# CaptainCuong/Efficient-GNN

Measured on NVIDIA B200. Metric: chebyshev_wavelet_nnz_k_f_per_s, higher is better.
Workload: dtype f32

## Files before the change

efficient-gnn_b200/_cabi.py:

```python
from __future__ import annotations

import ctypes as C
import os
import threading

_HERE = os.path.dirname(os.path.abspath(__file__))
LIB_PATH = os.environ.get("EGNN_LIB_PATH") or os.path.join(_HERE, "lib", "libegnn_b200.so")
ABI_VERSION = 8

_P, _I32, _I64, _F32, _SZ = C.c_void_p, C.c_int32, C.c_int64, C.c_float, C.c_size_t
SYMBOLS = {
    "egnn_abi_version": (C.c_int, []),
    "egnn_last_error": (C.c_char_p, []),
    "egnn_device_info": (C.c_int, [_P, _P, _P]),
    "egnn_dense_to_csr_count": (C.c_int, [_P, _I64, _I64, _P, _P, _P]),
    "egnn_dense_to_csr_fill": (C.c_int, [_P, _I64, _I64, _P, _P, _P, _P]),
    "egnn_graph_prep": (C.c_int, [_P, _P, _P, _I64, _P, _P, _P, _P, _P, _P, _P, _P, _P]),
    "egnn_degree_rows": (C.c_int, [_P, _P, _P, _I64, _I64, _I64, _P, _P, _P, _P, _P]),
    "egnn_graph_prep_finish": (C.c_int, [_P, _P, _P, _I64, _P, _P, _P, _P, _P]),
    "egnn_calibration_metrics_ws_bytes": (_SZ, [_I32, _I32]),
    "egnn_calibration_metrics": (C.c_int, [_P, _I32, _P, _P, _I64, _I32, _I32, _P, _P, _SZ, _P]),
    "egnn_temperature_head": (C.c_int, [_P, _P, _P, _P, _P, _P, _P, _P, _I64, _I32, _I32, _I32, _P]),
    "egnn_gcn_propagate": (C.c_int, [_P, _P, _P, _P, _P, _P, _P, _I64, _I32, _P, _P, _P, _I32, _P]),
    "egnn_gcn_target_logits": (C.c_int, [_P, _P, _P, _P, _P, _P, _I32, _I64, _I32, _I32, _P, _P, _P, _P, _P, _I32, _P]),
    "egnn_gcn_structure_grad": (C.c_int, [_P, _P, _P, _P, _P, _P, _P, _P, _P, _P, _I32, _I64, _I32, _I32, _P, _P,
                                          _P, _P, _P, _I32, _P]),
    "egnn_sell_geometry": (C.c_int, [_I64, _I64, _P, _P, _P]),
    "egnn_sell_ws_bytes": (_SZ, [_I64, _I64, _I32, _I32]),
    "egnn_sell_prepare": (C.c_int, [_P, _P, _I64, _I64, _P, _P, _SZ, _P]),
    "egnn_sell_fill": (C.c_int, [_P, _P, _I64, _I64, _P, _P, _SZ, _P]),
    "egnn_patch_degrees": (C.c_int, [_P, _P, _P, _P, _P, _I64, _P, _P, _P, _I32, _P, _P, _P, _I64, _I64, _P]),
# ... 22 lines not shown
                                         _F32, _F32, _I32, _P, _P, _P, _I32, _P, _P, _I32, _P, _P]),
    "egnn_peer_window_bytes": (_SZ, [_I64, _I32, _I32]),
    "egnn_peer_alloc": (C.c_int, [_SZ, _P, _P]),
    "egnn_peer_open": (C.c_int, [_P, _P]),
    "egnn_peer_close": (C.c_int, [_P]),
    "egnn_peer_free": (C.c_int, [_P]),
    "egnn_peer_operand": (_P, [_P, _I32]),
    "egnn_peer_error": (C.c_int, [_P, _P, _P]),
    "egnn_peer_wait_stats": (C.c_int, [_P, _P, _P, _I32, _P]),
    "egnn_peer_prescale_push": (C.c_int, [_P, _P, _I64, _I64, _I32, _P, _P]),
    "egnn_wide_order_sharded": (C.c_int, [_P, _P, _P, _P, _P, _P, _P, _P, _P, _I64, _I64, _I64, _I32, _I32, _I32, _I32,
                                          _P, _F32, _F32, _I32, _P, _P, _P, _I32, _P, _P]),
    "egnn_prescale": (C.c_int, [_P, _P, _P, _I64, _I32, _I64, _P]),
    "egnn_graph_prep_sharded": (C.c_int, [_P, _P, _P, _I64, _I64, _I64, _I32, _P, _P, _P, _P, _P, _P, _P, _P, _P]),
    "egnn_cheb_order_sharded": (C.c_int, [_P, _P, _P, _P, _P, _P, _P, _P, _P, _P, _P, _P,
                                          _I64, _I64, _I64, _I64, _I32, _I32, _I32, _I32, _P, _F32, _F32,
                                          _I32, _I32, _P, _P, _P, _I32, _P]),
}


class SellPlanStruct(C.Structure):
    _fields_ = [("n", C.c_int32), ("n_blocks", C.c_int32), ("col_block", C.c_int32), ("lmax", C.c_int32),
                ("n_cols", C.c_int32), ("row0", C.c_int32), ("n_cta", C.c_int32), ("reserved", C.c_int32),
                ("n_slices", C.c_int64), ("n_vrows", C.c_int64), ("n_entries", C.c_int64), ("n_rowv", C.c_int64),
                ("slice_off", C.c_void_p), ("blk_slice_ptr", C.c_void_p), ("idx", C.c_void_p),
                ("rv_ptr", C.c_void_p), ("vslot", C.c_void_p), ("cta_info", C.c_void_p), ("vpart", C.c_void_p),
                ("sched", C.c_void_p), ("stamps", C.c_void_p)]


MAX_RANKS = 16
IPC_HANDLE_BYTES = 64


class PeerWindowStruct(C.Structure):
    _fields_ = [("rank", C.c_int32), ("world", C.c_int32), ("rows_per", C.c_int64), ("f", C.c_int32),
                ("reserved", C.c_int32), ("base", C.c_void_p * MAX_RANKS)]


class EgnnError(RuntimeError):
    """A non-zero status from libegnn_b200 (message from egnn_last_error)."""


_lock = threading.Lock()
_lib = None


# ... 68 lines not shown
```

efficient-gnn_b200/csrc/egnn_cabi.cu:

```cuda
#include <stdarg.h>
#include <stdlib.h>

#include "adjoint.cuh"
#include "cheb.cuh"
#include "common.cuh"
#include "head.cuh"
#include "metrics.cuh"
#include "peer.cuh"
#include "prep.cuh"
#include "sell.cuh"
#include "sell_step.cuh"
#include "structure_grad.cuh"
#include "surrogate.cuh"
#include "blocked.cuh"
#include "wide.cuh"

namespace egnn {

static thread_local char g_err[512] = {0};
char* last_error_buf() { return g_err; }
void set_error(const char* fmt, ...) {
    va_list ap;
    va_start(ap, fmt);
    vsnprintf(g_err, sizeof(g_err), fmt, ap);
// ... 216 lines not shown
    EGNN_REQUIRE(w->world >= 1 && w->world <= EGNN_MAX_RANKS && w->rank >= 0 && w->rank < w->world, "bad rank/world");
    EGNN_REQUIRE(w->rows_per >= 1 && w->f >= 1, "bad window shape");
    for (int r = 0; r < w->world; ++r) EGNN_REQUIRE(w->base[r] != nullptr, "window of a rank is not mapped");
    return EGNN_OK;
}
static void fill_peer_push(PeerPush& pp, const egnn_peer_window* w, int which, bool has_data, bool wait_first) {
    pp.world = w->world; pp.rank = w->rank; pp.wait_first = wait_first; pp.has_data = has_data;
    char* own = (char*)w->base[w->rank];
    for (int r = 0; r < w->world; ++r) {
        pp.dst[r] = peer_operand(w, r, which);
        pp.flag[r] = (unsigned*)((char*)w->base[r] + kPeerFlagsOff) + w->rank;
    }
    pp.local_flags = (unsigned*)(own + kPeerFlagsOff);
    pp.epoch = (unsigned*)(own + kPeerEpochOff);
    pp.done_ctr = (unsigned*)(own + kPeerDoneOff);
    pp.error = (unsigned*)(own + kPeerErrorOff);
}

static void step_fill_plan(SellStepParams& sp, const egnn_sell_plan* pl) {
    sp.idx = pl->idx; sp.slice_off = pl->slice_off; sp.blk_slice_ptr = pl->blk_slice_ptr; sp.vslot = pl->vslot;
    sp.cta_info = pl->cta_info; sp.rv_ptr = pl->rv_ptr; sp.vpart = pl->vpart; sp.sched = pl->sched;
    sp.stamps = (unsigned long long*)pl->stamps;
    sp.trace = pl->reserved;
    sp.n_cta = pl->n_cta; sp.C = pl->n_blocks; sp.CB = pl->col_block; sp.n_cols = pl->n_cols;
    sp.n_rows = pl->n; sp.row0 = pl->row0;
}

static void step_fill_peer(SellStepParams& sp, const egnn_peer_window* w) {
    sp.world = w->world; sp.rank = w->rank; sp.rows_per = w->rows_per;
    char* own = (char*)w->base[w->rank];
    for (int r = 0; r < w->world; ++r) sp.flag_at[r] = (unsigned*)((char*)w->base[r] + kPeerFlagsOff) + w->rank;
    sp.local_flags = (unsigned*)(own + kPeerFlagsOff);
    sp.epoch = (unsigned*)(own + kPeerEpochOff);
    sp.error = (unsigned*)(own + kPeerErrorOff);
}

static int launch_sell_step(const SellStepParams& sp, bool peer, cudaStream_t st) {
    const size_t smem = sizeof(float) * ((size_t)sp.CB + kSellZeroSlots);
    const bool patch = sp.w_base != nullptr && sp.delta.n > 0;
    const void* fn = peer ? (patch ? (const void*)sell_step_kernel<true, true> : (const void*)sell_step_kernel<true, false>)
                          : (patch ? (const void*)sell_step_kernel<false, true> : (const void*)sell_step_kernel<false, false>);
    int rc = check_cuda(cudaFuncSetAttribute(fn, cudaFuncAttributeMaxDynamicSharedMemorySize, (int)smem),
                        "cudaFuncSetAttribute(sell_step_kernel)");
    if (rc) return rc;
    cudaLaunchConfig_t cfg = {};
    cfg.gridDim = dim3((unsigned)sp.n_cta, 1, 1);
    cfg.blockDim = dim3(kSellThreads, 1, 1);
    cfg.dynamicSmemBytes = smem;
    cfg.stream = st;
    cudaLaunchAttribute attr[1];
    attr[0].id = cudaLaunchAttributeCooperative;
    attr[0].val.cooperative = 1;
    cfg.attrs = attr;
    cfg.numAttrs = 1;
    void* args[1] = {(void*)&sp};
    return check_cuda(cudaLaunchKernelExC(&cfg, fn, args), "sell_step_kernel launch");
}

static int run_sell_step(SellStepParams sp, int k, int n_scales, const float* coeffs_host, bool peer, cudaStream_t st,
                         int order_begin = 1, int order_end = -1) {
    if (order_end < 0) order_end = k;
    const float* held = sp.operand_first;
    for (int ob = order_begin; ob <= order_end; ob += kStepMaxOrders) {
        const int oe = ob + kStepMaxOrders - 1 < order_end ? ob + kStepMaxOrders - 1 : order_end;
        sp.order_begin = ob; sp.order_end = oe; sp.k_max = k; sp.S = n_scales;
        sp.operand_first = ob == order_begin ? held : nullptr;
        for (int s = 0; s < n_scales; ++s)
            for (int j = 0; j <= oe - ob + 1; ++j) sp.coef[s][j] = coeffs_host[s * (k + 1) + ob - 1 + j];
        int rc = launch_sell_step(sp, peer, st);
        if (rc) return rc;
    }
    return EGNN_OK;
}

static int device_sm_count() {
    int dev = 0, sms = kSmCountB200;
    if (cudaGetDevice(&dev) == cudaSuccess) cudaDeviceGetAttribute(&sms, cudaDevAttrMultiProcessorCount, dev);
    return sms;
}

}

using namespace egnn;

extern "C" {

int egnn_abi_version(void) { return 8; }

const char* egnn_last_error(void) { return last_error_buf(); }

int egnn_device_info(int32_t* sm_count, int32_t* cc_major, int32_t* cc_minor) {
    int dev = 0;
    int rc = check_cuda(cudaGetDevice(&dev), "cudaGetDevice");
    if (rc) return rc;
    cudaDeviceProp prop;
    rc = check_cuda(cudaGetDeviceProperties(&prop, dev), "cudaGetDeviceProperties");
    if (rc) return rc;
    if (sm_count) *sm_count = prop.multiProcessorCount;
    if (cc_major) *cc_major = prop.major;
    if (cc_minor) *cc_minor = prop.minor;
    if (prop.major != 10) {
        set_error("libegnn_b200 is built for sm_100a only; device is sm_%d%d", prop.major, prop.minor);
        return EGNN_ERR_UNSUPPORTED_ARCH;
    }
    return EGNN_OK;
}

int egnn_dense_to_csr_count(const float* adj, int64_t n, int64_t ld, int32_t* rowptr,
                            int32_t* nonbinary, egnn_stream_t stream) {
    EGNN_REQUIRE(adj && rowptr && nonbinary, "null pointer");
// ... 844 lines not shown

int egnn_sell_geometry(int64_t n, int64_t nnz, int32_t* n_blocks, int32_t* col_block, int32_t* lmax) {
    EGNN_REQUIRE(n_blocks && col_block && lmax, "null pointer");
    EGNN_REQUIRE(n >= 1, "bad shape");
    int nb = 1, cb = 32;
    narrow_geometry(n, &nb, &cb);
    *n_blocks = nb;
    *col_block = cb;
    *lmax = 256;
    (void)nnz;
    return EGNN_OK;
}

size_t egnn_sell_ws_bytes(int64_t n, int64_t nnz, int32_t n_blocks, int32_t lmax) {
    if (n < 1 || n_blocks < 1 || lmax < 8) return 0;
    return sell_ws_layout(nullptr, n, nnz, n_blocks, lmax).total_bytes;
}

int egnn_sell_prepare(const int32_t* rowptr, const int32_t* colidx, int64_t n, int64_t nnz,
                      egnn_sell_plan* plan, void* workspace, size_t workspace_bytes, egnn_stream_t stream) {
    int rc = sell_check_geometry(n, nnz, plan);
    if (rc) return rc;
    EGNN_REQUIRE(rowptr && (colidx || nnz == 0), "null pointer");
    const int C = plan->n_blocks, CB = plan->col_block, lmax = plan->lmax;
    SellWs w = sell_ws_layout(workspace, n, nnz, C, lmax);
    if (!workspace || workspace_bytes < w.total_bytes) {
        set_error("sell workspace too small: need %zu bytes, got %zu", w.total_bytes, workspace_bytes);
        return EGNN_ERR_WORKSPACE;
    }
    cudaStream_t st = (cudaStream_t)stream;
    const int64_t cn = (int64_t)C * n;
    rc = check_cuda(cudaMemsetAsync(w.nv + cn, 0, 4, st), "memset"); if (rc) return rc;
    rc = check_cuda(cudaMemsetAsync(w.nvrow + n, 0, 4, st), "memset"); if (rc) return rc;
    rc = check_cuda(cudaMemsetAsync(w.key, 0xff, 4 * w.umax, st), "memset"); if (rc) return rc;
    rc = check_cuda(cudaMemsetAsync(w.slice_sz, 0, 4 * (w.smax + 1), st), "memset"); if (rc) return rc;
    rc = check_cuda(cudaMemsetAsync(w.totals, 0, 64, st), "memset"); if (rc) return rc;
    sell_count_kernel<<<(unsigned)ceil_div64(n, 256), 256, 0, st>>>(rowptr, colidx, (int)n, C, CB, lmax, w.seg_start,
                                                                   w.seg_cnt, w.nv, w.nvrow);
    EGNN_LAUNCH_CHECK("sell_count_kernel launch");
    size_t tb = w.cub_bytes;
    rc = check_cuda(cub::DeviceScan::ExclusiveSum(w.cub_temp, tb, w.nv, w.u_off, (int)(cn + 1), st), "scan nv"); if (rc) return rc;
    tb = w.cub_bytes;
    rc = check_cuda(cub::DeviceScan::ExclusiveSum(w.cub_temp, tb, w.nvrow, w.rv_ptr, (int)(n + 1), st), "scan nvrow"); if (rc) return rc;
    sell_emit_kernel<<<(unsigned)ceil_div64(cn, 256), 256, 0, st>>>((int)n, C, lmax, w.seg_start, w.seg_cnt, w.nv, w.u_off,
                                                                   w.rv_ptr, w.key, w.uval, w.vsrc, w.vslot, w.vrow);
    EGNN_LAUNCH_CHECK("sell_emit_kernel launch");
    tb = w.cub_bytes;
    rc = check_cuda(cub::DeviceRadixSort::SortPairs(w.cub_temp, tb, w.key, w.key_sorted, w.uval, w.perm, (int)w.umax, 0, 32, st), "sort vrows");
    if (rc) return rc;
    sell_blocks_kernel<<<1, 32, 0, st>>>((int)n, C, w.u_off, w.q_ptr, w.vp_ptr, w.bsp, w.bstride, w.totals);
    EGNN_LAUNCH_CHECK("sell_blocks_kernel launch");
    sell_slice_kernel<<<(unsigned)ceil_div64(w.smax, 256), 256, 0, st>>>(C, lmax, w.key_sorted, w.q_ptr, w.bsp, w.bstride, w.totals, w.slice_sz);
    EGNN_LAUNCH_CHECK("sell_slice_kernel launch");
    tb = w.cub_bytes;
    rc = check_cuda(cub::DeviceScan::ExclusiveSum(w.cub_temp, tb, w.slice_sz, w.slice_off, (int)(w.smax + 1), st), "scan slices"); if (rc) return rc;
    sell_totals_kernel<<<1, 32, 0, st>>>(w.slice_off, w.rv_ptr, (int)n, w.totals);
    EGNN_LAUNCH_CHECK("sell_totals_kernel launch");
    int64_t tot[8];
    rc = check_cuda(cudaMemcpyAsync(tot, w.totals, 64, cudaMemcpyDeviceToHost, st), "copy totals"); if (rc) return rc;
    rc = check_cuda(cudaStreamSynchronize(st), "sync"); if (rc) return rc;
    plan->n = (int32_t)n;
    plan->n_cta = device_sm_count();
    plan->n_vrows = tot[kTotV];
    plan->n_slices = tot[kTotSlices];
    plan->n_entries = tot[kTotEntries];
    plan->n_rowv = tot[kTotRowV];
    return EGNN_OK;
}

int egnn_sell_fill(const int32_t* rowptr, const int32_t* colidx, int64_t n, int64_t nnz,
                   const egnn_sell_plan* plan, void* workspace, size_t workspace_bytes, egnn_stream_t stream) {
    int rc = sell_check_geometry(n, nnz, plan);
    if (rc) return rc;
    (void)rowptr;
    EGNN_REQUIRE(plan->slice_off && plan->blk_slice_ptr && plan->rv_ptr && plan->cta_info && plan->sched, "plan buffers not allocated");
    EGNN_REQUIRE(plan->n_cta >= 1 && plan->n_cta <= 4096, "n_cta out of range");
    EGNN_REQUIRE(plan->n_entries == 0 || plan->idx, "plan idx not allocated");
    EGNN_REQUIRE(plan->n_vrows == 0 || plan->vslot, "plan vslot not allocated");
    const int C = plan->n_blocks, CB = plan->col_block, lmax = plan->lmax;
    SellWs w = sell_ws_layout(workspace, n, nnz, C, lmax);
    if (!workspace || workspace_bytes < w.total_bytes) {
        set_error("sell workspace too small: need %zu bytes, got %zu", w.total_bytes, workspace_bytes);
        return EGNN_ERR_WORKSPACE;
    }
    cudaStream_t st = (cudaStream_t)stream;
    rc = check_cuda(cudaMemcpyAsync(plan->slice_off, w.slice_off, 4 * (plan->n_slices + 1), cudaMemcpyDeviceToDevice, st), "copy slice_off"); if (rc) return rc;
    rc = check_cuda(cudaMemcpyAsync(plan->blk_slice_ptr, w.bsp, 4 * (C + 1), cudaMemcpyDeviceToDevice, st), "copy blk_slice_ptr"); if (rc) return rc;
    rc = check_cuda(cudaMemcpyAsync(plan->rv_ptr, w.rv_ptr, 4 * (n + 1), cudaMemcpyDeviceToDevice, st), "copy rv_ptr"); if (rc) return rc;
    sell_cta_blocks_kernel<<<1, 32, 0, st>>>(w.slice_off, w.bsp, C, plan->n_cta, plan->cta_info, plan->sched);
    EGNN_LAUNCH_CHECK("sell_cta_blocks_kernel launch");
    sell_row_cost_kernel<<<(unsigned)ceil_div64(n + 1, 256), 256, 0, st>>>(w.rv_ptr, (int)n, w.nvrow);
    EGNN_LAUNCH_CHECK("sell_row_cost_kernel launch");
    size_t tb = w.cub_bytes;
    rc = check_cuda(cub::DeviceScan::ExclusiveSum(w.cub_temp, tb, w.nvrow, w.nv, (int)(n + 1), st), "scan row costs"); if (rc) return rc;
    sell_cta_rows_kernel<<<(unsigned)ceil_div64(plan->n_cta + 1, 128), 128, 0, st>>>(w.nv, (int)n, plan->n_cta,
                                                                                 plan->cta_info + 2 * plan->n_cta + kSellMaxBlocks);
    EGNN_LAUNCH_CHECK("sell_cta_rows_kernel launch");
    if (plan->n_slices > 0) {
        rc = check_cuda(cudaFuncSetAttribute(sell_fill_kernel, cudaFuncAttributeMaxDynamicSharedMemorySize, (int)kSellFillSmem),
                        "cudaFuncSetAttribute(sell_fill_kernel)");
        if (rc) return rc;
        sell_fill_kernel<<<(unsigned)ceil_div64(plan->n_slices, kSellFillWarps), kSellFillWarps * 32, kSellFillSmem, st>>>(
            colidx, C, CB, lmax, (int)plan->n_slices, w.key_sorted, w.perm, w.vsrc, w.vslot, w.vrow, w.q_ptr, w.vp_ptr,
            w.bsp, w.bstride, w.slice_off, plan->idx, plan->vslot, plan->row0);
        EGNN_LAUNCH_CHECK("sell_fill_kernel launch");
    }
    return EGNN_OK;
}

int egnn_sell_step_sharded(const egnn_sell_plan* plan, const float* dinv_full, const uint8_t* iso_full,
                           const float* x0_local, const float* y_first_full, float* y_slab0, float* y_slab1,
                           float* tbuf0, float* tbuf1, float* t_all_or_null, float* out_local,
// ... 396 lines not shown
```

efficient-gnn_b200/csrc/sell.cuh:

```cuda
#pragma once

#include <cub/device/device_radix_sort.cuh>
#include <cub/device/device_scan.cuh>

#include "cheb.cuh"
#include "common.cuh"
#include "peer.cuh"

namespace egnn {

constexpr int kSellThreads = 1024;
constexpr int kSellThreadsPerCta = kSellThreads;
constexpr int kSellCtrStride = 32;
constexpr int kSellSchedWords = 64 * kSellCtrStride + 64;
constexpr int kSellSliceRows = 32;
constexpr int kSellGroup = 8;
constexpr int kSellMaxBlocks = 64;

enum SellTotals { kTotU = 0, kTotV = 1, kTotSlices = 2, kTotEntries = 3, kTotRowV = 4 };

__global__ void __launch_bounds__(256)
sell_count_kernel(const int32_t* __restrict__ rowptr, const int32_t* __restrict__ colidx, int n, int C,
                  int CB, int lmax, int32_t* __restrict__ seg_start, int32_t* __restrict__ seg_cnt,
                  int32_t* __restrict__ nv, int32_t* __restrict__ nvrow) {
// ... 80 lines not shown
    while (c + 1 < C && s >= blk_slice_ptr[c + 1]) ++c;
    return c;
}

__device__ __forceinline__ int sell_rank_of_slice(const int32_t* blk_slice_ptr, const int32_t* blk_stride, int c, int s) {
    const int n_c = blk_slice_ptr[c + 1] - blk_slice_ptr[c];
    return (int)(((int64_t)(s - blk_slice_ptr[c]) * blk_stride[c]) % n_c);
}

__global__ void __launch_bounds__(256)
sell_slice_kernel(int C, int lmax, const uint32_t* __restrict__ key_sorted,
                  const int32_t* __restrict__ q_ptr, const int32_t* __restrict__ blk_slice_ptr,
                  const int32_t* __restrict__ blk_stride, const int64_t* __restrict__ totals,
                  int32_t* __restrict__ slice_sz) {
    const int s = blockIdx.x * blockDim.x + threadIdx.x;
    if (s >= (int)totals[kTotSlices]) return;
    const int c = sell_block_of_slice(blk_slice_ptr, C, s);
    const int rank0 = sell_rank_of_slice(blk_slice_ptr, blk_stride, c, s) * kSellSliceRows;
    const int len = lmax - (int)(key_sorted[q_ptr[c] + rank0] & 0xffffu);
    slice_sz[s] = (len + kSellGroup - 1) / kSellGroup * kSellGroup * kSellSliceRows;
}

__global__ void sell_cta_blocks_kernel(const int32_t* __restrict__ slice_off, const int32_t* __restrict__ blk_slice_ptr,
                                       int C, int n_cta, int32_t* __restrict__ cta_info, unsigned* __restrict__ sched) {
    if (threadIdx.x != 0 || blockIdx.x != 0) return;
    double w[kSellMaxBlocks], total = 0.0;
    int cnt[kSellMaxBlocks];
    for (int c = 0; c < C; ++c) {
        w[c] = (double)(slice_off[blk_slice_ptr[c + 1]] - slice_off[blk_slice_ptr[c]]);
        total += w[c];
    }
    int used = 0;
    for (int c = 0; c < C; ++c) {
        cnt[c] = w[c] > 0 ? max(1, (int)(w[c] / total * n_cta)) : 0;
        used += cnt[c];
    }
    while (used > n_cta) {
        int big = 0;
        for (int c = 1; c < C; ++c) if (cnt[c] > cnt[big]) big = c;
        --cnt[big]; --used;
    }
    while (used < n_cta && total > 0) {
        int best = -1;
        double best_load = 0.0;
        for (int c = 0; c < C; ++c)
            if (cnt[c] > 0 && w[c] / cnt[c] > best_load) { best_load = w[c] / cnt[c]; best = c; }
        if (best < 0) break;
        ++cnt[best]; ++used;
    }
    int g = 0, max_cnt = 0;
    for (int c = 0; c < C; ++c) max_cnt = max(max_cnt, cnt[c]);
    for (int r = 0; r < max_cnt; ++r)
        for (int c = 0; c < C; ++c)
            if (r < cnt[c]) { cta_info[g] = c; cta_info[n_cta + g] = r; ++g; }
    for (; g < n_cta; ++g) { cta_info[g] = -1; cta_info[n_cta + g] = 0; }
    for (int i = 0; i < kSellSchedWords; ++i) sched[i] = 0u;
    for (int c = 0; c < kSellMaxBlocks; ++c) {
        const int start = c < C ? cnt[c] * (kSellThreadsPerCta / 32) : 0;
        cta_info[2 * n_cta + c] = start;
        sched[c * kSellCtrStride] = (unsigned)start;
    }
}

constexpr int kSellEpiWarpRow = 24;
__global__ void sell_row_cost_kernel(const int32_t* __restrict__ rv_ptr, int n, int32_t* __restrict__ cost) {
    const int i = blockIdx.x * blockDim.x + threadIdx.x;
    if (i > n) return;
    if (i == n) { cost[i] = 0; return; }
    const int parts = rv_ptr[i + 1] - rv_ptr[i];
    cost[i] = parts > kSellEpiWarpRow ? 28 + parts / 8 : 4;
}

__global__ void sell_cta_rows_kernel(const int32_t* __restrict__ cost_prefix, int n, int n_cta, int32_t* __restrict__ cta_rows) {
    const int g = blockIdx.x * blockDim.x + threadIdx.x;
    if (g > n_cta) return;
    if (g == 0) { cta_rows[0] = 0; return; }
    if (g == n_cta) { cta_rows[g] = n; return; }
    const int64_t target = (int64_t)cost_prefix[n] * g / n_cta;
    int lo = 0, hi = n;
    while (lo < hi) {
        const int mid = (lo + hi) >> 1;
// ... 131 lines not shown
```

efficient-gnn_b200/csrc/sell_step.cuh:

```cuda
#pragma once

#include "common.cuh"
#include "peer.cuh"
#include "prep.cuh"
#include "sell.cuh"

namespace egnn {

constexpr int kStepMaxOrders = 16;
constexpr int kSchedBarrier = kSellMaxBlocks * kSellCtrStride;
constexpr int kEpiWarpRow = kSellEpiWarpRow;
constexpr int kStageChunkFloats = 8192;

struct SellStepParams {
    const uint16_t* idx;
    const int32_t* slice_off;
    const int32_t* blk_slice_ptr;
    const int32_t* vslot;
    const int32_t* cta_info;
    const int32_t* rv_ptr;
    float* vpart;
    unsigned* sched;
    unsigned long long* stamps;
    int32_t trace;
    int32_t n_cta, C, CB, n_cols, n_rows, row0;
    const float* dinv;
    const uint8_t* iso;
    const float* x0;
    const float* operand_first;
    const float* operand[2];
    float* ydst[2][EGNN_MAX_RANKS];
    int32_t n_dst;
    float* tbuf[2];
    float* t_all;
    float* out;
    int32_t order_begin, order_end, k_max, S, normalize;
    float a, b;
    float coef[EGNN_MAX_SCALES][kStepMaxOrders + 1];
    DeltaList delta;
    const float* w_base;
    const float* rowsum_base;
    int32_t patch_x0;
    int32_t world, rank;
    int64_t rows_per;
    unsigned* flag_at[EGNN_MAX_RANKS];
    unsigned* local_flags;
    unsigned* epoch;
    unsigned* error;
// ... 1 lines not shown

__device__ __forceinline__ unsigned smem_u32(const void* p) { return (unsigned)__cvta_generic_to_shared(p); }
__device__ __forceinline__ void mbar_init(unsigned long long* bar, unsigned count) {
    asm volatile("mbarrier.init.shared::cta.b64 [%0], %1;" ::"r"(smem_u32(bar)), "r"(count) : "memory");
    asm volatile("fence.mbarrier_init.release.cluster;" ::: "memory");
}
__device__ __forceinline__ void mbar_expect_tx(unsigned long long* bar, unsigned bytes) {
    asm volatile("mbarrier.arrive.expect_tx.shared::cta.b64 _, [%0], %1;" ::"r"(smem_u32(bar)), "r"(bytes) : "memory");
}
__device__ __forceinline__ void mbar_wait(unsigned long long* bar, unsigned parity) {
    asm volatile(
        "{\n\t.reg .pred p;\n\t"
        "WAIT_LOOP:\n\t"
        "mbarrier.try_wait.parity.shared::cta.b64 p, [%0], %1;\n\t"
        "@p bra WAIT_DONE;\n\t"
        "bra WAIT_LOOP;\n\t"
        "WAIT_DONE:\n\t}"
        ::"r"(smem_u32(bar)), "r"(parity) : "memory");
}
__device__ __forceinline__ void bulk_g2s(void* dst_smem, const void* src, unsigned bytes, unsigned long long* bar) {
    asm volatile("cp.async.bulk.shared::cluster.global.mbarrier::complete_tx::bytes [%0], [%1], %2, [%3];"
                 ::"r"(smem_u32(dst_smem)), "l"(src), "r"(bytes), "r"(smem_u32(bar)) : "memory");
}
__device__ __forceinline__ void fence_proxy_async() { asm volatile("fence.proxy.async;" ::: "memory"); }

__device__ __forceinline__ unsigned long long ld_relaxed_gpu_u64(const unsigned long long* p) {
    unsigned long long v;
    asm volatile("ld.relaxed.gpu.global.u64 %0, [%1];" : "=l"(v) : "l"(p) : "memory");
    return v;
}
__device__ __forceinline__ void grid_arrive(unsigned long long* ctr, bool sys_scope) {
    if (sys_scope) __threadfence_system(); else __threadfence();
    atomicAdd(ctr, 1ull);
}
__device__ __forceinline__ void grid_wait(const unsigned long long* ctr, unsigned long long target) {
    while ((long long)(ld_relaxed_gpu_u64(ctr) - target) < 0) { }
    __threadfence();
}

__device__ __forceinline__ void peer_wait_ranks(const unsigned* local_flags, int p_lo, int p_hi, int rank,
                                                unsigned epoch, unsigned* error, bool stats, int lane) {
    const unsigned long long t0 = global_timer_ns();
    for (int p = p_lo + lane; p <= p_hi; p += 32) {
        if (p == rank) continue;
        while ((int)(ld_relaxed_sys_u32(local_flags + p) - epoch) < 0) {
            __nanosleep(32);
            if (global_timer_ns() - t0 > kPeerTimeoutNs) {
                atomicExch(error, 1u);
                break;
            }
        }
    }
    __syncwarp();
    if (lane == 0) __threadfence_system();
    __syncwarp();
    if (stats && lane == 0) {
        unsigned long long* stat = reinterpret_cast<unsigned long long*>(
            reinterpret_cast<char*>(const_cast<unsigned*>(local_flags)) - kPeerFlagsOff + kPeerWaitNsOff);
        stat[0] += global_timer_ns() - t0;
        stat[1] += 1ull;
// ... 148 lines not shown
        if (tid < n_touch) {
            const int u = tid < p.delta.n ? p.delta.row[tid] : p.delta.col[tid - p.delta.n];
            float dw = 0.f, dr = 0.f;
            for (int j = 0; j < p.delta.n; ++j) {
                if (p.delta.col[j] == u && p.delta.row[j] != u) dw += p.delta.val[j];
                if (p.delta.row[j] == u) dr += p.delta.val[j];
            }
            float dv;
            uint8_t is;
            normaliser_from_w(__ldg(p.w_base + u) + dw, dv, is);
            const int lr = u - p.row0;
            float x = 0.f;
            if (p.patch_x0) x = (float)log1p((double)(__ldg(p.rowsum_base + u) + dr));
            else if (lr >= 0 && lr < p.n_rows) x = __ldg(p.x0 + lr);
            pt_node[tid] = u; pt_dinv[tid] = dv; pt_iso[tid] = is; pt_x0[tid] = x; pt_y0[tid] = dv * x;
            if (p.t_all && p.order_begin == 1 && lr >= r0 && lr < r1) p.t_all[lr] = x;
        }
        for (int d = 0; d < p.delta.n; ++d) {
            const int a = p.delta.row[d] - p.row0, b = p.delta.col[d] - p.row0;
            touched_here |= (a >= r0 && a < r1) || (b >= r0 && b < r1);
        }
    }
    __syncthreads();

    auto wait_windows_free = [&]() {
        if (PEER && wid == 0) peer_wait_ranks(p.local_flags, 0, p.world - 1, p.rank, epoch_base + signals, p.error, false, lane);
    };
    auto signal_peers = [&]() {
        signals += 1u;
        if (PEER && g == 0 && tid == 0) {
            const unsigned e = epoch_base + signals;
            *p.epoch = e;
            __threadfence_system();
            for (int q = 0; q < p.world; ++q)
                if (q != p.rank) st_relaxed_sys_u32(p.flag_at[q], e);
        }
    };
    auto stamp = [&]() {
        if (p.stamps && g == 0 && tid == 0) p.stamps[stamp_i] = global_timer_ns();
        ++stamp_i;
    };
    int trace_i = 0;
    auto trace = [&]() {
        if (p.stamps && p.trace && tid == 0 && trace_i < 64) p.stamps[64 + (size_t)g * 64 + trace_i] = global_timer_ns();
        ++trace_i;
    };
// ... 37 lines not shown
        StepOrderView v;
        v.k = k; v.j = k - p.order_begin; v.flips_here = flips_here; v.flip_term = flip_term;
        v.touched_here = touched_here; v.n_touch = n_touch;
        v.pt_node = pt_node; v.pt_dinv = pt_dinv; v.pt_x0 = pt_x0; v.pt_iso = pt_iso;
        v.first = k == 1; v.last = k == p.k_max; v.push = k < p.k_max;
        const bool held = (k == p.order_begin) && p.operand_first != nullptr;
        v.operand = held ? p.operand_first : p.operand[(k - 1) & 1];
        v.tprev = step_t_ptr(p, k - 1);
        v.tprev2 = k >= 2 ? step_t_ptr(p, k - 2) : nullptr;
        v.tk = p.t_all ? p.t_all + (size_t)k * p.n_rows : (v.last ? nullptr : p.tbuf[(k - 1) & 1]);

        int s = bs1, off = 0, end = 0, slot = -1;
        if (has_slices) {
            s = bs0 + wid * ctas_in_block + rank_in_block;
            if (s < bs1) {
                off = __ldg(p.slice_off + s);
                end = __ldg(p.slice_off + s + 1);
                slot = __ldg(p.vslot + (size_t)s * kSellSliceRows + lane);
                const char* head = reinterpret_cast<const char*>(p.idx + off) + lane * 128;
                if (head < reinterpret_cast<const char*>(p.idx + end)) asm volatile("prefetch.global.L2 [%0];" ::"l"(head));
            }
        }
        finish_pending();
        if (has_slices) {
            unsigned raw_next = 0;
            if (lane == 0) raw_next = atomicAdd(p.sched + c * kSellCtrStride, 1u);
            const float* src = v.operand + col0;
            const int cnt4 = cnt & ~3;
            if (wid == 0) {
                if (PEER && !held) {
                    const int p_lo = (int)(col0 / p.rows_per);
                    const int p_hi = (int)((col0 + cnt - 1) / p.rows_per);
                    peer_wait_ranks(p.local_flags, p_lo, min(p_hi, p.world - 1), p.rank, epoch_base + signals, p.error,
                                    g == 0, lane);
                }
                if (lane == 0) {
                    fence_proxy_async();
                    if (cnt4 > 0) {
                        mbar_expect_tx(&stage_bar, (unsigned)cnt4 * 4u);
                        for (int o = 0; o < cnt4; o += kStageChunkFloats)
                            bulk_g2s(ysm + o, src + o, (unsigned)min(kStageChunkFloats, cnt4 - o) * 4u, &stage_bar);
                    }
                }
            }
            if (PEER && !held) __syncthreads();
            if (tid >= 32) {
                for (int t = cnt4 + tid - 32; t < p.CB + kSellZeroSlots; t += kSellThreads - 32)
                    ysm[t] = t < cnt ? __ldcg(src + t) : 0.f;
            }
            if (cnt4 > 0) mbar_wait(&stage_bar, stage_parity);
            stage_parity ^= (cnt4 > 0) ? 1u : 0u;
            __syncthreads();
            if (PATCH && held && k == 1) {
                if (tid < n_touch) {
                    const int loc = pt_node[tid] - col0;
                    if (loc >= 0 && loc < cnt) ysm[loc] = pt_y0[tid];
                }
                __syncthreads();
            }
            trace();

            while (s < bs1) {
                int s_next = bs0 + (int)__shfl_sync(0xffffffffu, raw_next, 0);
                if (lane == 0) raw_next = atomicAdd(p.sched + c * kSellCtrStride, 1u);
// ... 44 lines not shown
        bar_wait();
        stamp();
        if (PEER && v.last && !late_done) signal_peers();
        if (g == 0 && tid < p.C) p.sched[tid * kSellCtrStride] = (unsigned)__ldg(p.cta_info + 2 * p.n_cta + tid);
        for (int i = i_a; i < r1; i += kSellThreads) {
            const StepRowPre r = i == i_a ? pre_a : (i == i_b ? pre_b : step_row_prefetch<PATCH>(p, v, i));
            if (r.e - r.t > kEpiWarpRow) {
                const int h = atomicAdd(&hub_cnt, 1);
                if (h < hub_cap) { hub_list[h] = i; continue; }
            }
            step_epilogue_finish(p, v, i, r, step_row_sum(p.vpart, r.t, r.e));
        }
        __syncthreads();
        const int n_hub = min(hub_cnt, hub_cap);
        for (int h = wid; h < n_hub; h += kWarps) {
            const int i = hub_list[h];
            const StepRowPre r = step_row_prefetch<PATCH>(p, v, i);
            double a = 0.0;
            for (int t = r.t + lane; t < r.e; t += 32) a += (double)__ldcg(p.vpart + t);
#pragma unroll
            for (int o = 16; o > 0; o >>= 1) a += __shfl_xor_sync(0xffffffffu, a, o);
            if (lane == 0) step_epilogue_finish(p, v, i, r, a);
        }
        if (k < p.order_end || (PEER && (v.push || (v.last && late_done)))) {
            bar_arrive(PEER && v.push);
            pending = true; pending_signal = v.push || (v.last && late_done);
        }
        trace();
    }
    finish_pending();
    if (p.stamps && g == 0 && tid == 0) p.stamps[stamp_i] = global_timer_ns();
}

}
```

efficient-gnn_b200/graph.py:

```python
from __future__ import annotations

import ctypes as C
from typing import Optional, Sequence

import numpy as np
import torch

from . import _cabi

__all__ = ["CsrGraph", "as_graph", "deltas_from_dense", "enable_phase_stamps", "read_phase_stamps"]


def _stream():
    return _cabi.current_stream()


class CsrGraph:

    def __init__(self, rowptr: torch.Tensor, colidx: torch.Tensor, vals: Optional[torch.Tensor], n: int,
                 _prepare: bool = True):
        _cabi.require_device()
        if rowptr.dtype != torch.int32 or colidx.dtype != torch.int32:
            raise TypeError("rowptr/colidx must be int32")
        if not (rowptr.is_cuda and colidx.is_cuda):
            raise _cabi.EgnnError("CsrGraph arrays must live on the CUDA device")
# ... 258 lines not shown

    def patch_nodes(self, deltas, restore: bool = False):
        if self._scratch is None:
            self._scratch = (self.dinv.clone(), self.iso.clone(), self.x0.clone(), self.y0().clone())
        d_rows, d_cols, d_vals = deltas
        lib = _cabi.load()
        with torch.cuda.device(self.device):
            _cabi.check(lib.egnn_patch_nodes(
                _cabi.ptr(self.w), _cabi.ptr(self.rowsum), _cabi.ptr(self.dinv), _cabi.ptr(self.iso), _cabi.ptr(self.x0),
                _cabi.ptr(self.y0()), self.n,
                _cabi.host_array(C.c_int32, [int(v) for v in d_rows]),
                _cabi.host_array(C.c_int32, [int(v) for v in d_cols]),
                _cabi.host_array(C.c_float, [float(v) for v in d_vals]), len(d_rows),
                *[_cabi.ptr(t) for t in self._scratch], 1 if restore else 0, _stream()), "egnn_patch_nodes")
        return self._scratch

    def to_scipy(self):
        import scipy.sparse as sp
        data = np.ones(self.nnz, np.float32) if self.vals is None else self.vals.cpu().numpy()
        return sp.csr_matrix((data, self.colidx.cpu().numpy(), self.rowptr.cpu().numpy()),
                             shape=(self.n, self.n))


def build_sell_plan(rowptr: torch.Tensor, colidx: torch.Tensor, n_rows: int, n_cols: int, row0: int, geometry):
    lib = _cabi.load()
    dev = rowptr.device
    nnz = int(colidx.numel())
    nb, cb, lmax = geometry
    with torch.cuda.device(dev):
        plan = _cabi.SellPlanStruct()
        plan.n, plan.n_blocks, plan.col_block, plan.lmax = n_rows, nb, cb, lmax
        plan.n_cols, plan.row0 = n_cols, row0
        ws_bytes = int(lib.egnn_sell_ws_bytes(n_rows, nnz, nb, lmax))
        ws = torch.empty(ws_bytes, dtype=torch.uint8, device=dev)
        _cabi.check(lib.egnn_sell_prepare(_cabi.ptr(rowptr), _cabi.ptr(colidx), n_rows, nnz,
                                          C.byref(plan), _cabi.ptr(ws), ws_bytes, _stream()), "egnn_sell_prepare")
        bufs = {
            "slice_off": torch.empty(plan.n_slices + 1, dtype=torch.int32, device=dev),
            "blk_slice_ptr": torch.empty(plan.n_blocks + 1, dtype=torch.int32, device=dev),
            "idx": torch.empty(max(1, plan.n_entries), dtype=torch.int16, device=dev),
            "rv_ptr": torch.empty(n_rows + 1, dtype=torch.int32, device=dev),
            "vslot": torch.empty(max(1, plan.n_vrows), dtype=torch.int32, device=dev),
            "cta_info": torch.empty(3 * plan.n_cta + 65, dtype=torch.int32, device=dev),
            "vpart": torch.empty(max(1, plan.n_rowv), dtype=torch.float32, device=dev),
            "sched": torch.zeros(64 * 32 + 64, dtype=torch.int32, device=dev),
        }
        for name, t in bufs.items():
            setattr(plan, name, t.data_ptr())
        _cabi.check(lib.egnn_sell_fill(_cabi.ptr(rowptr), _cabi.ptr(colidx), n_rows, nnz,
                                       C.byref(plan), _cabi.ptr(ws), ws_bytes, _stream()), "egnn_sell_fill")
    plan._keepalive = bufs
    return plan


def enable_phase_stamps(plan, on: bool = True, trace: bool = False):
# ... 65 lines not shown
```

include/egnn_b200.h:

```cpp
#ifndef EGNN_B200_H
#define EGNN_B200_H

#include <stddef.h>
#include <stdint.h>

#ifdef __cplusplus
extern "C" {
#endif

typedef void* egnn_stream_t;

enum egnn_status {
    EGNN_OK = 0,
    EGNN_ERR_INVALID_ARG = -1,
    EGNN_ERR_CUDA = -2,
    EGNN_ERR_UNSUPPORTED_ARCH = -3,
    EGNN_ERR_WORKSPACE = -4
};

#define EGNN_MAX_SCALES 8
#define EGNN_MAX_ORDER 64
#define EGNN_MAX_DELTA 64
#define EGNN_MAX_RANKS 16
#define EGNN_IPC_HANDLE_BYTES 64
// ... 25 lines not shown
int egnn_graph_prep_finish(const double* colsum, const float* diag, const float* rowsum,
                           int64_t n, float* dinv, uint8_t* iso, float* x0_logdeg,
                           float* w_out_or_null, egnn_stream_t stream);

int egnn_patch_degrees(const float* w_base, const float* rowsum_base,
                       const float* dinv_base, const uint8_t* iso_base,
                       const float* x0_base, int64_t n,
                       const int32_t* delta_row_host, const int32_t* delta_col_host,
                       const float* delta_val_host, int32_t n_delta,
                       float* dinv_out, uint8_t* iso_out, float* x0_out,
                       int64_t row_begin, int64_t n_rows, egnn_stream_t stream);

int egnn_patch_nodes(const float* w_base, const float* rowsum_base, const float* dinv_base,
                     const uint8_t* iso_base, const float* x0_base, const float* y0_base, int64_t n,
                     const int32_t* delta_row_host, const int32_t* delta_col_host,
                     const float* delta_val_host, int32_t n_delta,
                     float* dinv_io, uint8_t* iso_io, float* x0_io, float* y0_io,
                     int32_t restore, egnn_stream_t stream);

typedef struct egnn_sell_plan {
    int32_t n, n_blocks, col_block, lmax;
    int32_t n_cols, row0;
    int32_t n_cta, reserved;
    int64_t n_slices, n_vrows, n_entries, n_rowv;
    int32_t* slice_off;
    int32_t* blk_slice_ptr;
    uint16_t* idx;
    int32_t* rv_ptr;
    int32_t* vslot;
    int32_t* cta_info;
    float* vpart;
    uint32_t* sched;
    uint64_t* stamps;
} egnn_sell_plan;

int egnn_sell_geometry(int64_t n_cols, int64_t nnz, int32_t* n_blocks, int32_t* col_block, int32_t* lmax);
size_t egnn_sell_ws_bytes(int64_t n, int64_t nnz, int32_t n_blocks, int32_t lmax);
int egnn_sell_prepare(const int32_t* rowptr, const int32_t* colidx, int64_t n, int64_t nnz,
                      egnn_sell_plan* plan, void* workspace, size_t workspace_bytes,
                      egnn_stream_t stream);
int egnn_sell_fill(const int32_t* rowptr, const int32_t* colidx, int64_t n, int64_t nnz,
                   const egnn_sell_plan* plan, void* workspace, size_t workspace_bytes,
                   egnn_stream_t stream);

size_t egnn_cheb_workspace_bytes(int64_t n, int32_t f);
int egnn_cheb_wavelet(const int32_t* rowptr, const int32_t* colidx,
// ... 174 lines not shown
```

Measured before the change: 2073 billion.

## Add optional thread-block-cluster multicast staging and release/acquire grid barrier to SELL step

Adds an optional cluster launch for the cooperative SELL step kernel. CTAs in a cluster split the bulk copy of the column-block vector and use TMA multicast, so each slice of the vector is fetched from global memory once per cluster rather than once per CTA. The CTA scheduler is changed to hand out work in cluster-sized units, and cluster barriers protect reuse of the shared staging buffer. Separately, the device-scope grid barrier now uses a red.release add and ld.acquire polling instead of a full __threadfence plus atomicAdd and relaxed polling. With default settings the cluster size is 1, so only the barrier change and cheap cluster-size checks take effect.

```diff
diff --git a/efficient-gnn_b200/_cabi.py b/efficient-gnn_b200/_cabi.py
--- a/efficient-gnn_b200/_cabi.py
+++ b/efficient-gnn_b200/_cabi.py
@@ -6,7 +6,7 @@
 
 _HERE = os.path.dirname(os.path.abspath(__file__))
 LIB_PATH = os.environ.get("EGNN_LIB_PATH") or os.path.join(_HERE, "lib", "libegnn_b200.so")
-ABI_VERSION = 8
+ABI_VERSION = 9
 
 _P, _I32, _I64, _F32, _SZ = C.c_void_p, C.c_int32, C.c_int64, C.c_float, C.c_size_t
 SYMBOLS = {
@@ -75,6 +75,7 @@
 class SellPlanStruct(C.Structure):
     _fields_ = [("n", C.c_int32), ("n_blocks", C.c_int32), ("col_block", C.c_int32), ("lmax", C.c_int32),
                 ("n_cols", C.c_int32), ("row0", C.c_int32), ("n_cta", C.c_int32), ("reserved", C.c_int32),
+                ("cluster", C.c_int32), ("reserved2", C.c_int32),
                 ("n_slices", C.c_int64), ("n_vrows", C.c_int64), ("n_entries", C.c_int64), ("n_rowv", C.c_int64),
                 ("slice_off", C.c_void_p), ("blk_slice_ptr", C.c_void_p), ("idx", C.c_void_p),
                 ("rv_ptr", C.c_void_p), ("vslot", C.c_void_p), ("cta_info", C.c_void_p), ("vpart", C.c_void_p),
diff --git a/efficient-gnn_b200/csrc/egnn_cabi.cu b/efficient-gnn_b200/csrc/egnn_cabi.cu
--- a/efficient-gnn_b200/csrc/egnn_cabi.cu
+++ b/efficient-gnn_b200/csrc/egnn_cabi.cu
@@ -262,7 +262,7 @@
     sp.cta_info = pl->cta_info; sp.rv_ptr = pl->rv_ptr; sp.vpart = pl->vpart; sp.sched = pl->sched;
     sp.stamps = (unsigned long long*)pl->stamps;
     sp.trace = pl->reserved;
-    sp.n_cta = pl->n_cta; sp.C = pl->n_blocks; sp.CB = pl->col_block; sp.n_cols = pl->n_cols;
+    sp.n_cta = pl->n_cta; sp.cluster = pl->cluster; sp.C = pl->n_blocks; sp.CB = pl->col_block; sp.n_cols = pl->n_cols;
     sp.n_rows = pl->n; sp.row0 = pl->row0;
 }
 
@@ -275,26 +275,64 @@
     sp.error = (unsigned*)(own + kPeerErrorOff);
 }
 
+constexpr int kStepClusterDefault = 1;
+
+static size_t sell_step_smem(int CB) { return sizeof(float) * ((size_t)CB + kSellZeroSlots); }
+
+static cudaLaunchConfig_t sell_step_config(int n_cta, int cluster, size_t smem, cudaStream_t st, cudaLaunchAttribute* attr) {
+    cudaLaunchConfig_t cfg = {};
+    cfg.gridDim = dim3((unsigned)n_cta, 1, 1);
+    cfg.blockDim = dim3(kSellThreads, 1, 1);
+    cfg.dynamicSmemBytes = smem;
+    cfg.stream = st;
+    attr[0].id = cudaLaunchAttributeCooperative;
+    attr[0].val.cooperative = 1;
+    cfg.attrs = attr;
+    cfg.numAttrs = 1;
+    if (cluster > 1) {
+        attr[1].id = cudaLaunchAttributeClusterDimension;
+        attr[1].val.clusterDim.x = (unsigned)cluster;
+        attr[1].val.clusterDim.y = 1;
+        attr[1].val.clusterDim.z = 1;
+        cfg.numAttrs = 2;
+    }
+    return cfg;
+}
+
 static int launch_sell_step(const SellStepParams& sp, bool peer, cudaStream_t st) {
-    const size_t smem = sizeof(float) * ((size_t)sp.CB + kSellZeroSlots);
+    const size_t smem = sell_step_smem(sp.CB);
     const bool patch = sp.w_base != nullptr && sp.delta.n > 0;
     const void* fn = peer ? (patch ? (const void*)sell_step_kernel<true, true> : (const void*)sell_step_kernel<true, false>)
                           : (patch ? (const void*)sell_step_kernel<false, true> : (const void*)sell_step_kernel<false, false>);
     int rc = check_cuda(cudaFuncSetAttribute(fn, cudaFuncAttributeMaxDynamicSharedMemorySize, (int)smem),
                         "cudaFuncSetAttribute(sell_step_kernel)");
     if (rc) return rc;
-    cudaLaunchConfig_t cfg = {};
-    cfg.gridDim = dim3((unsigned)sp.n_cta, 1, 1);
-    cfg.blockDim = dim3(kSellThreads, 1, 1);
-    cfg.dynamicSmemBytes = smem;
-    cfg.stream = st;
-    cudaLaunchAttribute attr[1];
-    attr[0].id = cudaLaunchAttributeCooperative;
-    attr[0].val.cooperative = 1;
-    cfg.attrs = attr;
-    cfg.numAttrs = 1;
+    cudaLaunchAttribute attr[2];
+    const cudaLaunchConfig_t cfg = sell_step_config(sp.n_cta, sp.cluster, smem, st, attr);
     void* args[1] = {(void*)&sp};
     return check_cuda(cudaLaunchKernelExC(&cfg, fn, args), "sell_step_kernel launch");
+}
+
+static void sell_step_grid(int want, int C, int CB, int* n_cta, int* cluster) {
+    const int sms = device_sm_count();
+    const int cl = want > 0 ? want : kStepClusterDefault;
+    *n_cta = sms;
+    *cluster = 1;
+    if (cl <= 1) return;
+    const void* fn = (const void*)sell_step_kernel<false, false>;
+    const size_t smem = sell_step_smem(CB);
+    int fit = 0;
+    if (cudaFuncSetAttribute(fn, cudaFuncAttributeMaxDynamicSharedMemorySize, (int)smem) == cudaSuccess) {
+        cudaLaunchAttribute attr[2];
+        const cudaLaunchConfig_t cfg = sell_step_config(sms / cl * cl, cl, smem, 0, attr);
+        if (cudaOccupancyMaxActiveClusters(&fit, fn, &cfg) != cudaSuccess) fit = 0;
+    }
+    (void)cudaGetLastError();
+    const int units = fit < sms / cl ? fit : sms / cl;
+    if (units >= 1 && units >= C) {
+        *n_cta = units * cl;
+        *cluster = cl;
+    }
 }
 
 static int run_sell_step(SellStepParams sp, int k, int n_scales, const float* coeffs_host, bool peer, cudaStream_t st,
@@ -325,7 +363,7 @@
 
 extern "C" {
 
-int egnn_abi_version(void) { return 8; }
+int egnn_abi_version(void) { return 9; }
 
 const char* egnn_last_error(void) { return last_error_buf(); }
 
@@ -1216,6 +1254,8 @@
     int rc = sell_check_geometry(n, nnz, plan);
     if (rc) return rc;
     EGNN_REQUIRE(rowptr && (colidx || nnz == 0), "null pointer");
+    EGNN_REQUIRE(plan->cluster >= 0 && plan->cluster <= 16 && (plan->cluster & (plan->cluster - 1)) == 0,
+                 "cluster must be 0 (default) or a power of two up to 16");
     const int C = plan->n_blocks, CB = plan->col_block, lmax = plan->lmax;
     SellWs w = sell_ws_layout(workspace, n, nnz, C, lmax);
     if (!workspace || workspace_bytes < w.total_bytes) {
@@ -1254,7 +1294,7 @@
     rc = check_cuda(cudaMemcpyAsync(tot, w.totals, 64, cudaMemcpyDeviceToHost, st), "copy totals"); if (rc) return rc;
     rc = check_cuda(cudaStreamSynchronize(st), "sync"); if (rc) return rc;
     plan->n = (int32_t)n;
-    plan->n_cta = device_sm_count();
+    sell_step_grid(plan->cluster, C, CB, &plan->n_cta, &plan->cluster);
     plan->n_vrows = tot[kTotV];
     plan->n_slices = tot[kTotSlices];
     plan->n_entries = tot[kTotEntries];
@@ -1269,6 +1309,9 @@
     (void)rowptr;
     EGNN_REQUIRE(plan->slice_off && plan->blk_slice_ptr && plan->rv_ptr && plan->cta_info && plan->sched, "plan buffers not allocated");
     EGNN_REQUIRE(plan->n_cta >= 1 && plan->n_cta <= 4096, "n_cta out of range");
+    EGNN_REQUIRE(plan->cluster >= 1 && plan->n_cta % plan->cluster == 0 &&
+                 (plan->cluster == 1 || plan->n_cta / plan->cluster >= plan->n_blocks),
+                 "cluster must divide n_cta into at least n_blocks clusters (egnn_sell_prepare chooses it)");
     EGNN_REQUIRE(plan->n_entries == 0 || plan->idx, "plan idx not allocated");
     EGNN_REQUIRE(plan->n_vrows == 0 || plan->vslot, "plan vslot not allocated");
     const int C = plan->n_blocks, CB = plan->col_block, lmax = plan->lmax;
@@ -1281,7 +1324,7 @@
     rc = check_cuda(cudaMemcpyAsync(plan->slice_off, w.slice_off, 4 * (plan->n_slices + 1), cudaMemcpyDeviceToDevice, st), "copy slice_off"); if (rc) return rc;
     rc = check_cuda(cudaMemcpyAsync(plan->blk_slice_ptr, w.bsp, 4 * (C + 1), cudaMemcpyDeviceToDevice, st), "copy blk_slice_ptr"); if (rc) return rc;
     rc = check_cuda(cudaMemcpyAsync(plan->rv_ptr, w.rv_ptr, 4 * (n + 1), cudaMemcpyDeviceToDevice, st), "copy rv_ptr"); if (rc) return rc;
-    sell_cta_blocks_kernel<<<1, 32, 0, st>>>(w.slice_off, w.bsp, C, plan->n_cta, plan->cta_info, plan->sched);
+    sell_cta_blocks_kernel<<<1, 32, 0, st>>>(w.slice_off, w.bsp, C, plan->n_cta, plan->cluster, plan->cta_info, plan->sched);
     EGNN_LAUNCH_CHECK("sell_cta_blocks_kernel launch");
     sell_row_cost_kernel<<<(unsigned)ceil_div64(n + 1, 256), 256, 0, st>>>(w.rv_ptr, (int)n, w.nvrow);
     EGNN_LAUNCH_CHECK("sell_row_cost_kernel launch");
diff --git a/efficient-gnn_b200/csrc/sell.cuh b/efficient-gnn_b200/csrc/sell.cuh
--- a/efficient-gnn_b200/csrc/sell.cuh
+++ b/efficient-gnn_b200/csrc/sell.cuh
@@ -126,25 +126,26 @@
 }
 
 __global__ void sell_cta_blocks_kernel(const int32_t* __restrict__ slice_off, const int32_t* __restrict__ blk_slice_ptr,
-                                       int C, int n_cta, int32_t* __restrict__ cta_info, unsigned* __restrict__ sched) {
+                                       int C, int n_cta, int cluster, int32_t* __restrict__ cta_info, unsigned* __restrict__ sched) {
     if (threadIdx.x != 0 || blockIdx.x != 0) return;
     double w[kSellMaxBlocks], total = 0.0;
     int cnt[kSellMaxBlocks];
+    const int n_units = n_cta / cluster;
     for (int c = 0; c < C; ++c) {
         w[c] = (double)(slice_off[blk_slice_ptr[c + 1]] - slice_off[blk_slice_ptr[c]]);
         total += w[c];
     }
     int used = 0;
     for (int c = 0; c < C; ++c) {
-        cnt[c] = w[c] > 0 ? max(1, (int)(w[c] / total * n_cta)) : 0;
+        cnt[c] = w[c] > 0 ? max(1, (int)(w[c] / total * n_units)) : 0;
         used += cnt[c];
     }
-    while (used > n_cta) {
+    while (used > n_units) {
         int big = 0;
         for (int c = 1; c < C; ++c) if (cnt[c] > cnt[big]) big = c;
         --cnt[big]; --used;
     }
-    while (used < n_cta && total > 0) {
+    while (used < n_units && total > 0) {
         int best = -1;
         double best_load = 0.0;
         for (int c = 0; c < C; ++c)
@@ -156,11 +157,12 @@
     for (int c = 0; c < C; ++c) max_cnt = max(max_cnt, cnt[c]);
     for (int r = 0; r < max_cnt; ++r)
         for (int c = 0; c < C; ++c)
-            if (r < cnt[c]) { cta_info[g] = c; cta_info[n_cta + g] = r; ++g; }
+            if (r < cnt[c])
+                for (int j = 0; j < cluster; ++j) { cta_info[g] = c; cta_info[n_cta + g] = r * cluster + j; ++g; }
     for (; g < n_cta; ++g) { cta_info[g] = -1; cta_info[n_cta + g] = 0; }
     for (int i = 0; i < kSellSchedWords; ++i) sched[i] = 0u;
     for (int c = 0; c < kSellMaxBlocks; ++c) {
-        const int start = c < C ? cnt[c] * (kSellThreadsPerCta / 32) : 0;
+        const int start = c < C ? cnt[c] * cluster * (kSellThreadsPerCta / 32) : 0;
         cta_info[2 * n_cta + c] = start;
         sched[c * kSellCtrStride] = (unsigned)start;
     }
diff --git a/efficient-gnn_b200/csrc/sell_step.cuh b/efficient-gnn_b200/csrc/sell_step.cuh
--- a/efficient-gnn_b200/csrc/sell_step.cuh
+++ b/efficient-gnn_b200/csrc/sell_step.cuh
@@ -23,7 +23,7 @@
     unsigned* sched;
     unsigned long long* stamps;
     int32_t trace;
-    int32_t n_cta, C, CB, n_cols, n_rows, row0;
+    int32_t n_cta, cluster, C, CB, n_cols, n_rows, row0;
     const float* dinv;
     const uint8_t* iso;
     const float* x0;
@@ -71,20 +71,45 @@
     asm volatile("cp.async.bulk.shared::cluster.global.mbarrier::complete_tx::bytes [%0], [%1], %2, [%3];"
                  ::"r"(smem_u32(dst_smem)), "l"(src), "r"(bytes), "r"(smem_u32(bar)) : "memory");
 }
+__device__ __forceinline__ void bulk_g2s_multicast(void* dst_smem, const void* src, unsigned bytes, unsigned long long* bar,
+                                                   unsigned short mask) {
+    asm volatile("cp.async.bulk.shared::cluster.global.mbarrier::complete_tx::bytes.multicast::cluster [%0], [%1], %2, [%3], %4;"
+                 ::"r"(smem_u32(dst_smem)), "l"(src), "r"(bytes), "r"(smem_u32(bar)), "h"(mask) : "memory");
+}
 __device__ __forceinline__ void fence_proxy_async() { asm volatile("fence.proxy.async;" ::: "memory"); }
+__device__ __forceinline__ unsigned cluster_size() {
+    unsigned r;
+    asm volatile("mov.u32 %0, %%cluster_nctarank;" : "=r"(r));
+    return r;
+}
+__device__ __forceinline__ unsigned cluster_rank() {
+    unsigned r;
+    asm volatile("mov.u32 %0, %%cluster_ctarank;" : "=r"(r));
+    return r;
+}
+__device__ __forceinline__ void cluster_arrive() { asm volatile("barrier.cluster.arrive.release.aligned;" ::: "memory"); }
+__device__ __forceinline__ void cluster_wait() { asm volatile("barrier.cluster.wait.acquire.aligned;" ::: "memory"); }
 
 __device__ __forceinline__ unsigned long long ld_relaxed_gpu_u64(const unsigned long long* p) {
     unsigned long long v;
     asm volatile("ld.relaxed.gpu.global.u64 %0, [%1];" : "=l"(v) : "l"(p) : "memory");
     return v;
 }
+__device__ __forceinline__ unsigned long long ld_acquire_gpu_u64(const unsigned long long* p) {
+    unsigned long long v;
+    asm volatile("ld.acquire.gpu.global.u64 %0, [%1];" : "=l"(v) : "l"(p) : "memory");
+    return v;
+}
 __device__ __forceinline__ void grid_arrive(unsigned long long* ctr, bool sys_scope) {
-    if (sys_scope) __threadfence_system(); else __threadfence();
-    atomicAdd(ctr, 1ull);
+    if (sys_scope) {
+        __threadfence_system();
+        atomicAdd(ctr, 1ull);
+    } else {
+        asm volatile("red.release.gpu.global.add.u64 [%0], 1;" ::"l"(ctr) : "memory");
+    }
 }
 __device__ __forceinline__ void grid_wait(const unsigned long long* ctr, unsigned long long target) {
-    while ((long long)(ld_relaxed_gpu_u64(ctr) - target) < 0) { }
-    __threadfence();
+    while ((long long)(ld_acquire_gpu_u64(ctr) - target) < 0) { }
 }
 
 __device__ __forceinline__ void peer_wait_ranks(const unsigned* local_flags, int p_lo, int p_hi, int rank,
@@ -279,6 +304,7 @@
         }
     }
     __syncthreads();
+    if (cluster_size() > 1) cluster_arrive();
 
     auto wait_windows_free = [&]() {
         if (PEER && wid == 0) peer_wait_ranks(p.local_flags, 0, p.world - 1, p.rank, epoch_base + signals, p.error, false, lane);
@@ -362,6 +388,7 @@
             }
         }
         finish_pending();
+        if (cluster_size() > 1) cluster_wait();
         if (has_slices) {
             unsigned raw_next = 0;
             if (lane == 0) raw_next = atomicAdd(p.sched + c * kSellCtrStride, 1u);
@@ -378,8 +405,16 @@
                     fence_proxy_async();
                     if (cnt4 > 0) {
                         mbar_expect_tx(&stage_bar, (unsigned)cnt4 * 4u);
-                        for (int o = 0; o < cnt4; o += kStageChunkFloats)
-                            bulk_g2s(ysm + o, src + o, (unsigned)min(kStageChunkFloats, cnt4 - o) * 4u, &stage_bar);
+                        const int cl = (int)cluster_size();
+                        if (cl == 1) {
+                            for (int o = 0; o < cnt4; o += kStageChunkFloats)
+                                bulk_g2s(ysm + o, src + o, (unsigned)min(kStageChunkFloats, cnt4 - o) * 4u, &stage_bar);
+                        } else {
+                            const unsigned short all = (unsigned short)((1u << cl) - 1u);
+                            for (int o = (int)cluster_rank() * kStageChunkFloats; o < cnt4; o += cl * kStageChunkFloats)
+                                bulk_g2s_multicast(ysm + o, src + o, (unsigned)min(kStageChunkFloats, cnt4 - o) * 4u,
+                                                   &stage_bar, all);
+                        }
                     }
                 }
             }
@@ -470,6 +505,7 @@
             for (int o = 16; o > 0; o >>= 1) a += __shfl_xor_sync(0xffffffffu, a, o);
             if (lane == 0) step_epilogue_finish(p, v, i, r, a);
         }
+        if (cluster_size() > 1) cluster_arrive();
         if (k < p.order_end || (PEER && (v.push || (v.last && late_done)))) {
             bar_arrive(PEER && v.push);
             pending = true; pending_signal = v.push || (v.last && late_done);
@@ -477,6 +513,7 @@
         trace();
     }
     finish_pending();
+    if (cluster_size() > 1) cluster_wait();
     if (p.stamps && g == 0 && tid == 0) p.stamps[stamp_i] = global_timer_ns();
 }
 
diff --git a/efficient-gnn_b200/graph.py b/efficient-gnn_b200/graph.py
--- a/efficient-gnn_b200/graph.py
+++ b/efficient-gnn_b200/graph.py
@@ -1,6 +1,7 @@
 from __future__ import annotations
 
 import ctypes as C
+import os
 from typing import Optional, Sequence
 
 import numpy as np
@@ -305,15 +306,19 @@
                              shape=(self.n, self.n))
 
 
-def build_sell_plan(rowptr: torch.Tensor, colidx: torch.Tensor, n_rows: int, n_cols: int, row0: int, geometry):
+def build_sell_plan(rowptr: torch.Tensor, colidx: torch.Tensor, n_rows: int, n_cols: int, row0: int, geometry,
+                    cluster: Optional[int] = None):
     lib = _cabi.load()
     dev = rowptr.device
     nnz = int(colidx.numel())
     nb, cb, lmax = geometry
+    if cluster is None:
+        cluster = int(os.environ.get("EGNN_STEP_CLUSTER", "0"))
     with torch.cuda.device(dev):
         plan = _cabi.SellPlanStruct()
         plan.n, plan.n_blocks, plan.col_block, plan.lmax = n_rows, nb, cb, lmax
         plan.n_cols, plan.row0 = n_cols, row0
+        plan.cluster = cluster
         ws_bytes = int(lib.egnn_sell_ws_bytes(n_rows, nnz, nb, lmax))
         ws = torch.empty(ws_bytes, dtype=torch.uint8, device=dev)
         _cabi.check(lib.egnn_sell_prepare(_cabi.ptr(rowptr), _cabi.ptr(colidx), n_rows, nnz,
diff --git a/include/egnn_b200.h b/include/egnn_b200.h
--- a/include/egnn_b200.h
+++ b/include/egnn_b200.h
@@ -71,6 +71,7 @@
     int32_t n, n_blocks, col_block, lmax;
     int32_t n_cols, row0;
     int32_t n_cta, reserved;
+    int32_t cluster, reserved2;
     int64_t n_slices, n_vrows, n_entries, n_rowv;
     int32_t* slice_off;
     int32_t* blk_slice_ptr;
```

Result: no change. 2089 billion, median of 6 (+0.8%).
